# nintendops/EPN_PointCloud

Hardware: AMD Instinct MI355X
Metric: point-clouds/sec fwd+bwd, ModelNet40 N=1024 A=60 (higher is better)
Workload: dtype f32

## Files before the change

### epn_pointcloud_amd/csrc/c_api.hip

```cpp
#include <atomic>
#include <cstdlib>
#include <cstring>
#include <cxxabi.h>

#include "conv_internal.h"

using namespace epn;

static std::atomic<int> g_policy{0};
static bool force_generic() { return g_policy.load(std::memory_order_relaxed) == 1; }

namespace epn {
bool first_layer_on_valu() { return g_policy.load(std::memory_order_relaxed) == 2; }
#ifdef EPN_TUNING
int kernel_policy() { return g_policy.load(std::memory_order_relaxed); }
#else
int kernel_policy() { return 0; }
#endif
}

namespace {
thread_local const void *t_stub = nullptr;
thread_local bool t_stub_aux = true;
}
namespace epn {
void note_kernel(const void *host_stub, bool aux) {
    if (aux && t_stub) return;
    t_stub = host_stub;
    t_stub_aux = aux;
}
}

extern "C" const char *epn_last_kernel(void) {
    static thread_local char out[320];
    out[0] = 0;
    const void *stub = t_stub;
    t_stub = nullptr;
    t_stub_aux = true;
    if (!stub) return out;
    const char *mangled = hipKernelNameRefByPtr(stub, nullptr);
    if (!mangled) return out;
    int status = 0;
    char *dem = abi::__cxa_demangle(mangled, nullptr, nullptr, &status);
    const char *b = (status == 0 && dem) ? dem : mangled;
    if (!std::strncmp(b, "void ", 5)) b += 5;
    static const char anon[] = "(anonymous namespace)::";
    size_t o = 0;
    int depth = 0;
    for (size_t i = 0; b[i] && o + 1 < sizeof(out);) {
        if (!std::strncmp(b + i, anon, sizeof(anon) - 1)) { i += sizeof(anon) - 1; continue; }
        if (b[i] == '<') ++depth;
        else if (b[i] == '>') --depth;
        else if (b[i] == '(' && depth == 0) break;
        out[o++] = b[i++];
    }
    out[o] = 0;
    std::free(dem);
    return out;
}

extern "C" int epn_set_kernel_policy(int policy) {
#ifdef EPN_TUNING
    if (policy != 0 && policy != 1 && policy != 2 && (policy & ~0xff) != 0x100 && (policy & ~0xff) != 0x200 && (policy & ~0xff) != 0x400 && (policy & ~0xff) != 0x800 && (policy & ~0xff) != 0x900) return EPN_EINVAL;
#else
    if (policy != 0 && policy != 1 && policy != 2) return EPN_EINVAL;
#endif
    g_policy.store(policy, std::memory_order_relaxed);
    return 0;
}

static int check_desc(const epn_inter_desc *d) {
    if (!d) return EPN_ENULL;
    if (d->b < 0 || d->p1 < 1 || d->p2 < 0 || d->nn < 1 || d->na < 1 || d->ks < 1 || d->cin < 1 || d->cout < 1)
        return EPN_EINVAL;
    if (d->ks > EPN_KS_GENERIC_MAX) return EPN_EINVAL;
    if (!(d->sigma > 0.f) && !d->dense_w) return EPN_EINVAL;
    if (!d->ball_idx) return EPN_ENULL;
    if (!d->dense_w && (!d->xyz || !d->new_xyz || !d->anchors || !d->kernels)) return EPN_ENULL;
    return 0;
}

static bool use_mfma(const epn_inter_desc *d) { return inter_uses_mfma(d) && !force_generic() && !d->dense_w; }

extern "C" const char *epn_version(void) { return "epn_so3conv 0.5 (gfx950)"; }
extern "C" int epn_abi_version(void) { return EPN_ABI_VERSION; }

extern "C" const char *epn_strerror(int code) {
    switch (code) {
        case 0: return "success";
        case EPN_EINVAL: return "epn: invalid size or unsupported shape";
        case EPN_EWORKSPACE: return "epn: workspace missing or too small";
        case EPN_ENULL: return "epn: required pointer is NULL";
        default: return code > 0 ? hipGetErrorString((hipError_t)code) : "epn: unknown error";
    }
}

extern "C" int epn_inter_is_fused(const epn_inter_desc *d) {
    return d && (use_mfma(d) || (inter_c1_fwd_ok(d) && !force_generic())) ? 1 : 0;
}

extern "C" int epn_intra_is_fused(int na, int kn, int cin, int cout) {
    return intra_uses_mfma(na, kn, cin, cout) && !force_generic() ? 1 : 0;
}

extern "C" size_t epn_inter_workspace_bytes(const epn_inter_desc *d) {
    if (!d) return 0;
    InterWs w = inter_ws(d);
    if (force_generic() || d->dense_w) {
        epn_inter_desc g = *d;
        g.cin = d->cin; g.cout = d->cout;
        const size_t big = (size_t)d->b * d->p2 * d->na * d->cin * d->ks;
        return (w.big_off + rnd64(big)) * sizeof(float);
    }
    return w.total_floats * sizeof(float);
}

static int prep(const epn_inter_desc *d, void *workspace, size_t bytes, bool need_big, InterWs &ws, float *&base,
                hipStream_t st, bool need_rk = true) {
    int rc = check_desc(d);
    if (rc) return rc;
    ws = inter_ws(d);
    const size_t big = need_big ? rnd64((size_t)d->b * d->p2 * d->na * d->cin * d->ks)
                                : ws.total_floats - ws.big_off;
    if (!workspace || bytes < (ws.big_off + big) * sizeof(float)) return EPN_EWORKSPACE;
    base = static_cast<float *>(workspace);
    if (!d->dense_w && need_rk) {
        rc = launch_rk_table(d, base + ws.rk_off, st);
        if (rc) return rc;
    }
    return 0;
}

extern "C" int epn_inter_weights_f32(const epn_inter_desc *d, float *w, epn_stream_t stream) {
    int rc = check_desc(d);
    if (rc) return rc;
    if (!w || !d->xyz || !d->new_xyz || !d->anchors || !d->kernels) return EPN_ENULL;
    if (d->b == 0 || d->p2 == 0) return 0;
    return launch_inter_weights(d, w, epn_stream(stream));
}

extern "C" int epn_inter_so3conv_fwd_f32(const epn_inter_desc *d, const float *feats_cl, const float *W,
                                         float *out_cl, void *workspace, size_t workspace_bytes,
                                         epn_stream_t stream) {
    hipStream_t st = epn_stream(stream);
    InterWs ws;
    float *base = nullptr;
    const bool mf = d && use_mfma(d);
    int rc = prep(d, workspace, workspace_bytes, !mf, ws, base, st, !mf);
    if (rc) return rc;
    if (!feats_cl || !W || !out_cl) return EPN_ENULL;
    if (d->b == 0 || d->p2 == 0) return 0;
    if (mf) {
        rc = launch_inter_tables_mfma(d, base + ws.rk4_off, st);
        if (rc) return rc;
        return launch_inter_fwd_mfma(d, base + ws.rk4_off, feats_cl, W, out_cl, st);
    }
    if (inter_c1_fwd_ok(d) && !force_generic())
        return launch_inter_c1_fwd(d, base + ws.rk_off, feats_cl, W, out_cl, st, nullptr,
                                   reinterpret_cast<unsigned *>(base + ws.beta_off));
    float *G = base + ws.big_off;
    rc = launch_inter_group(d, base + ws.rk_off, feats_cl, G, st);
    if (rc) return rc;
    return launch_rowgemm_nt(G, W, (size_t)d->b * d->p2 * d->na, d->cin * d->ks, d->cout, out_cl, st);
}

extern "C" int epn_inter_c1_ok(const epn_inter_desc *d) {
    return d && !check_desc(d) && inter_c1_fwd_ok(d) && inter_c1_bwd_weight_ok(d) && !force_generic() ? 1 : 0;
}
extern "C" int epn_inter_so3conv_fwd_c1_f32(const epn_inter_desc *d, const float *feats_cl, const float *W, float *out_cl,
                                            float *grouped, void *workspace, size_t workspace_bytes, epn_stream_t stream) {
    if (!epn_inter_c1_ok(d)) return EPN_EINVAL;
    hipStream_t st = epn_stream(stream);
    InterWs ws;
    float *base = nullptr;
    int rc = prep(d, workspace, workspace_bytes, false, ws, base, st);
    if (rc) return rc;
    if (!feats_cl || !W || !out_cl) return EPN_ENULL;
    if (d->b == 0 || d->p2 == 0) return 0;
    return launch_inter_c1_fwd(d, base + ws.rk_off, feats_cl, W, out_cl, st, grouped,
                               reinterpret_cast<unsigned *>(base + ws.beta_off));
}
extern "C" int epn_inter_so3conv_bwd_weight_c1_f32(const epn_inter_desc *d, const float *grouped, const float *grad_out_cl,
                                                   float *grad_W, epn_stream_t stream) {
    if (!epn_inter_c1_ok(d)) return EPN_EINVAL;
    if (!grad_W) return EPN_ENULL;
    hipStream_t st = epn_stream(stream);
    EPN_HIP(hipMemsetAsync(grad_W, 0, sizeof(float) * (size_t)d->cout * d->ks, st));
    if (d->b == 0 || d->p2 == 0) return 0;
    if (!grouped || !grad_out_cl) return EPN_ENULL;
    return launch_inter_c1_bwd_weight(d, nullptr, nullptr, grad_out_cl, grad_W, st, grouped);
}

extern "C" int epn_inter_so3conv_bwd_data_f32(const epn_inter_desc *d, const float *grad_out_cl, const float *W,
                                              float *grad_feats_cl, void *workspace, size_t workspace_bytes,
                                              epn_stream_t stream) {
    hipStream_t st = epn_stream(stream);
    InterWs ws;
    float *base = nullptr;
    const bool mf = d && use_mfma(d);
    int rc = prep(d, workspace, workspace_bytes, !mf, ws, base, st, !mf);
    if (rc) return rc;
    if (!grad_feats_cl) return EPN_ENULL;
    EPN_HIP(hipMemsetAsync(grad_feats_cl, 0, sizeof(float) * (size_t)d->b * d->p1 * d->na * d->cin, st));
    if (d->b == 0 || d->p2 == 0) return 0;
    if (!grad_out_cl || !W) return EPN_ENULL;
    if (mf) {
        rc = launch_inter_tables_mfma(d, base + ws.rk4_off, st);
        if (rc) return rc;
        return launch_inter_bwd_data_mfma(d, base + ws.rk4_off, base + ws.big_off, grad_out_cl, W, grad_feats_cl, st);
    }
    float *dG = base + ws.big_off;
    rc = launch_rowgemm_nn(grad_out_cl, W, (size_t)d->b * d->p2 * d->na, d->cin * d->ks, d->cout, dG, st);
    if (rc) return rc;
    return launch_inter_scatter(d, base + ws.rk_off, dG, grad_feats_cl, st);
}

extern "C" int epn_inter_so3conv_bwd_weight_f32(const epn_inter_desc *d, const float *feats_cl,
                                                const float *grad_out_cl, float *grad_W, void *workspace,
                                                size_t workspace_bytes, epn_stream_t stream) {
    hipStream_t st = epn_stream(stream);
    InterWs ws;
    float *base = nullptr;
    const bool mf = d && use_mfma(d);
    int rc = prep(d, workspace, workspace_bytes, !mf, ws, base, st, !mf);
    if (rc) return rc;
    if (!grad_W) return EPN_ENULL;
    EPN_HIP(hipMemsetAsync(grad_W, 0, sizeof(float) * (size_t)d->cout * d->cin * d->ks, st));
    if (d->b == 0 || d->p2 == 0) return 0;
    if (!feats_cl || !grad_out_cl) return EPN_ENULL;
    if (mf) {
        rc = launch_inter_tables_mfma(d, base + ws.rk4_off, st);
        if (rc) return rc;
        return launch_inter_bwd_weight_mfma(d, base + ws.rk4_off, feats_cl, grad_out_cl, grad_W, st);
    }
    if (inter_c1_bwd_weight_ok(d) && !force_generic())
        return launch_inter_c1_bwd_weight(d, base + ws.rk_off, feats_cl, grad_out_cl, grad_W, st);
    float *G = base + ws.big_off;
    rc = launch_inter_group(d, base + ws.rk_off, feats_cl, G, st);
    if (rc) return rc;
    return launch_colreduce_dw(grad_out_cl, G, (size_t)d->b * d->p2 * d->na, d->cin * d->ks, d->cout, grad_W, st);
}

extern "C" size_t epn_inter_group_workspace_bytes(const epn_inter_desc *d) {
    if (!d) return 0;
    InterWs w = inter_ws(d);
    return w.big_off * sizeof(float);
}

static int prep_tables(const epn_inter_desc *d, void *workspace, size_t bytes, InterWs &ws, float *&base,
                       hipStream_t st, bool need_rk = true) {
    int rc = check_desc(d);
    if (rc) return rc;
    if (d->dense_w) return EPN_EINVAL;
    ws = inter_ws(d);
    if (!workspace || bytes < ws.big_off * sizeof(float)) return EPN_EWORKSPACE;
    base = static_cast<float *>(workspace);
    return need_rk ? launch_rk_table(d, base + ws.rk_off, st) : 0;
}

extern "C" int epn_inter_onchip_ok(const epn_inter_desc *d, int bf16) {
    return d && !check_desc(d) && inter_fx_ok(d, bf16) && !force_generic() ? 1 : 0;
}

extern "C" size_t epn_inter_onchip_workspace_bytes(const epn_inter_desc *d, int bf16) {
    if (!d) return 0;
    InterWs w = inter_ws(d);
    return w.big_off * sizeof(float) + inter_fx_planes_bytes(d, bf16);
}

static int inter_onchip_fwd(const epn_inter_desc *d, const void *feats_cl, const float *W, void *out_cl, void *workspace,
                            size_t workspace_bytes, int bf16, epn_stream_t stream) {
    hipStream_t st = epn_stream(stream);
    int rc = check_desc(d);
    if (rc) return rc;
    if (!inter_fx_ok(d, bf16)) return EPN_EINVAL;
    if (workspace_bytes < epn_inter_onchip_workspace_bytes(d, bf16)) return EPN_EWORKSPACE;
    InterWs ws;
    float *base = nullptr;
    rc = prep_tables(d, workspace, workspace_bytes, ws, base, st, false);
    if (rc) return rc;
    if (d->b == 0 || d->p2 == 0) return 0;
    if (!feats_cl || !W || !out_cl) return EPN_ENULL;
    rc = launch_inter_tables_mfma(d, base + ws.rk4_off, st);
    if (rc) return rc;
    return launch_inter_fx_fwd(d, base + ws.rk4_off, feats_cl, W, out_cl, base + ws.big_off, bf16, st);
}

extern "C" int epn_inter_so3conv_fwd_onchip_f32(const epn_inter_desc *d, const float *feats_cl, const float *W,
                                                float *out_cl, void *workspace, size_t workspace_bytes,
                                                epn_stream_t stream) {
    return inter_onchip_fwd(d, feats_cl, W, out_cl, workspace, workspace_bytes, 0, stream);
}
extern "C" int epn_inter_so3conv_fwd_bf16(const epn_inter_desc *d, const void *feats_cl, const float *W, void *out_cl,
                                          void *workspace, size_t workspace_bytes, epn_stream_t stream) {
    return inter_onchip_fwd(d, feats_cl, W, out_cl, workspace, workspace_bytes, 1, stream);
}

static int inter_group_any(const epn_inter_desc *d, const void *feats_cl, void *grouped, void *workspace,
                           size_t workspace_bytes, int bf16, epn_stream_t stream, int packed = 0) {
    hipStream_t st = epn_stream(stream);
    InterWs ws;
    float *base = nullptr;
    int rc = prep_tables(d, workspace, workspace_bytes, ws, base, st, !(d && inter_group_mfma_ok(d) && !force_generic()));
    if (rc) return rc;
    if (d->b == 0 || d->p2 == 0) return 0;
    if (!feats_cl || !grouped) return EPN_ENULL;
    if (inter_group_mfma_ok(d) && !force_generic()) {
        rc = launch_inter_tables_mfma(d, base + ws.rk4_off, st);
        if (rc) return rc;
        return launch_inter_group_mfma(d, base + ws.rk4_off, feats_cl, grouped, bf16, st, packed);
    }
    if (bf16 || packed) return EPN_EINVAL;
    return launch_inter_group(d, base + ws.rk_off, static_cast<const float *>(feats_cl), static_cast<float *>(grouped), st);
}

static int inter_ungroup_any(const epn_inter_desc *d, const void *grad_grouped, float *grad_feats_cl, void *workspace,
                             size_t workspace_bytes, int bf16, epn_stream_t stream, bool accumulate = false) {
    hipStream_t st = epn_stream(stream);
    InterWs ws;
    float *base = nullptr;
    int rc = prep_tables(d, workspace, workspace_bytes, ws, base, st, !(d && inter_group_mfma_ok(d) && !force_generic()));
    if (rc) return rc;
    if (!grad_feats_cl) return EPN_ENULL;
    if (!accumulate)
        EPN_HIP(hipMemsetAsync(grad_feats_cl, 0, sizeof(float) * (size_t)d->b * d->p1 * d->na * d->cin, st));
    if (d->b == 0 || d->p2 == 0) return 0;
    if (!grad_grouped) return EPN_ENULL;
    if (inter_group_mfma_ok(d) && !force_generic()) {
        rc = launch_inter_tables_mfma(d, base + ws.rk4_off, st);
        if (rc) return rc;
        return launch_inter_ungroup_mfma(d, base + ws.rk4_off, grad_grouped, grad_feats_cl,
                                         reinterpret_cast<int32_t *>(base + ws.order_off), bf16, st);
    }
    if (bf16) return EPN_EINVAL;
    return launch_inter_scatter(d, base + ws.rk_off, static_cast<const float *>(grad_grouped), grad_feats_cl, st);
}

extern "C" int epn_inter_group_f32(const epn_inter_desc *d, const float *feats_cl, float *grouped, void *workspace,
                                   size_t workspace_bytes, epn_stream_t stream) {
    return inter_group_any(d, feats_cl, grouped, workspace, workspace_bytes, 0, stream);
}
extern "C" int epn_inter_group_bf16(const epn_inter_desc *d, const void *feats_cl, void *grouped, void *workspace,
                                    size_t workspace_bytes, epn_stream_t stream) {
    return inter_group_any(d, feats_cl, grouped, workspace, workspace_bytes, 1, stream);
}
extern "C" int epn_inter_group_packed_ok(const epn_inter_desc *d) {
    return d && !check_desc(d) && inter_group_packed_ok(d) && !force_generic() ? 1 : 0;
}
extern "C" int epn_inter_packed_position(int cin, int ks, int32_t *position) {
    if (cin < 32 || cin % 32 || ks < 4 || ks > EPN_KS_MAX || ks % 4) return EPN_EINVAL;
    if (!position) return EPN_ENULL;
    for (int c = 0; c < cin; ++c)
        for (int k = 0; k < ks; ++k) position[c * ks + k] = inter_packed_position(c, k, cin, ks);
    return 0;
}
extern "C" int epn_inter_group_packed_f32(const epn_inter_desc *d, const float *feats_cl, float *grouped, void *workspace,
                                          size_t workspace_bytes, epn_stream_t stream) {
    if (!epn_inter_group_packed_ok(d)) return EPN_EINVAL;
    return inter_group_any(d, feats_cl, grouped, workspace, workspace_bytes, 0, stream, 1);
}
extern "C" int epn_inter_group_packed_bf16(const epn_inter_desc *d, const void *feats_cl, void *grouped, void *workspace,
                                           size_t workspace_bytes, epn_stream_t stream) {
    if (!epn_inter_group_packed_ok(d)) return EPN_EINVAL;
    return inter_group_any(d, feats_cl, grouped, workspace, workspace_bytes, 1, stream, 1);
}
static int pack_args_ok(int cout, int cin, int ks) {
    return cout >= 0 && cin >= 32 && cin % 32 == 0 && ks >= 4 && ks <= EPN_KS_MAX && ks % 4 == 0;
}
// ... 224 lines not shown
```

### epn_pointcloud_amd/csrc/epn_common.h

```cpp
#pragma once
#include <hip/hip_runtime.h>
#include <stdint.h>

#include "../../include/epn_so3conv.h"

#define EPN_WAVE 64

#define EPN_CHECK_LAUNCH()                         \
    do {                                           \
        hipError_t _e = hipGetLastError();         \
        if (_e != hipSuccess) return (int)_e;      \
    } while (0)

#define EPN_HIP(call)                              \
    do {                                           \
        hipError_t _e = (call);                    \
        if (_e != hipSuccess) return (int)_e;      \
    } while (0)

static inline hipStream_t epn_stream(epn_stream_t s) { return (hipStream_t)s; }

namespace epn {
void note_kernel(const void *host_stub, bool aux);
bool first_layer_on_valu();
}
#define EPN_LAUNCH(kern, ...)                                                       \
    do {                                                                            \
        ::epn::note_kernel(reinterpret_cast<const void *>(&kern), false);           \
        hipLaunchKernelGGL(kern, __VA_ARGS__);                                      \
    } while (0)
#define EPN_LAUNCH_AUX(kern, ...)                                                   \
    do {                                                                            \
        ::epn::note_kernel(reinterpret_cast<const void *>(&kern), true);            \
        hipLaunchKernelGGL(kern, __VA_ARGS__);                                      \
    } while (0)

static inline int epn_cdiv(long long a, long long b) { return (int)((a + b - 1) / b); }

__device__ __forceinline__ float epn_sq3(float a, float b, float c) {
    float t = __fmul_rn(a, a);
    t = __fmaf_rn(b, b, t);
    t = __fmaf_rn(c, c, t);
    return t;
}

__device__ __forceinline__ unsigned epn_xcd_tile(unsigned bid, unsigned nb) {
    const unsigned xcd = bid & 7u, local = bid >> 3;
    const unsigned q = nb >> 3, r = nb & 7u;
    return (xcd < r ? xcd * (q + 1) : r * (q + 1) + (xcd - r) * q) + local;
}

typedef float f32x4 __attribute__((ext_vector_type(4)));
typedef float f32x16 __attribute__((ext_vector_type(16)));
```

### epn_pointcloud_amd/csrc/inter_ungroup_cloud.hip

```cpp
#include "inter_device.h"
#include "gemm.h"

namespace epn {
namespace {

__device__ unsigned g_uc_range = 0u;

constexpr int UC_DUMMY = 4;
constexpr int UC_LDS_MAX = 160 * 1024;

constexpr int UC_PTS = 8;
__global__ __launch_bounds__(256) void uc_slots_kernel(const int32_t *__restrict__ idx, const float *__restrict__ xyz,
                                                       const float *__restrict__ new_xyz, long long npts, int p1, int p2, int nn, int ew,
                                                       float sigma_inv, unsigned rowb, uint32_t *__restrict__ off,
                                                       float *__restrict__ hood, unsigned *__restrict__ mulmax) {
    const int lane = threadIdx.x & 63;
    const long long pt0 = ((long long)blockIdx.x * 4 + (threadIdx.x >> 6)) * UC_PTS;
    if (pt0 >= npts) return;
    const bool in = lane < nn;
    int q[UC_PTS];
#pragma unroll
    for (int i = 0; i < UC_PTS; ++i) {
        const long long pt = pt0 + i < npts ? pt0 + i : npts - 1;
        q[i] = in ? idx[pt * nn + lane] : -1;
    }
    bool valid[UC_PTS];
    unsigned mul[UC_PTS];
    float g[UC_PTS][3], cc[UC_PTS][3];
#pragma unroll
    for (int i = 0; i < UC_PTS; ++i) {
        const long long pt = pt0 + i < npts ? pt0 + i : npts - 1;
        const long long bb = pt / p2;
        const int pp = (int)(pt - bb * p2);
        const int first = __shfl(q[i], 0, 64);
        const unsigned long long rep = __ballot(in && lane > 0 && q[i] == first);
        int cnt = rep ? (int)__builtin_ctzll(rep) : nn;
        const int qprev = __shfl(q[i], lane >= cnt ? lane - cnt : lane, 64);
        const bool bad = in && lane >= cnt && q[i] != qprev;
        if (__ballot(bad) != 0ull) cnt = nn;
        valid[i] = q[i] >= 0 && q[i] < p1;
        mul[i] = (valid[i] && lane < cnt) ? (unsigned)((nn - 1 - lane) / cnt + 1) : 0u;
        const float *s = xyz + bb * 3 * p1, *c = new_xyz + bb * 3 * p2;
        const int qq = valid[i] ? q[i] : 0;
        g[i][0] = s[qq]; g[i][1] = s[p1 + qq]; g[i][2] = s[2 * p1 + qq];
        cc[i][0] = c[pp]; cc[i][1] = c[p2 + pp]; cc[i][2] = c[2 * p2 + pp];
    }
    unsigned m = 0;
#pragma unroll
    for (int i = 0; i < UC_PTS; ++i) {
        const long long pt = pt0 + i < npts ? pt0 + i : npts - 1;
        if (lane < ew) {
            off[pt * ew + lane] = (valid[i] ? (unsigned)q[i] : (unsigned)(p1 + ((lane >> 2) & 3))) * rowb;
            const float gx = g[i][0] - cc[i][0], gy = g[i][1] - cc[i][1], gz = g[i][2] - cc[i][2];
            const float alpha = 1.0f - (gx * gx + gy * gy + gz * gz) * sigma_inv;
            const float mf = (float)mul[i];
            float *h = hood + pt * 5 * ew + lane;
            h[0] = gx * mf; h[ew] = gy * mf; h[2 * ew] = gz * mf; h[3 * ew] = mf; h[4 * ew] = alpha * mf;
        }
        m = mul[i] > m ? mul[i] : m;
    }
#pragma unroll
    for (int o = 32; o >= 1; o >>= 1) {
        const unsigned v = (unsigned)__shfl_xor((int)m, o, 64);
        m = v > m ? v : m;
    }
    if (lane == 0 && m > 1u && m > __atomic_load_n(mulmax, __ATOMIC_RELAXED)) atomicMax(mulmax, m);
}

template <typename TG>
__global__ __launch_bounds__(256) void uc_absmax_kernel(const TG *__restrict__ src, long long n, unsigned *__restrict__ out) {
    unsigned m = 0;
    for (long long i = (long long)blockIdx.x * 256 + threadIdx.x; i < n; i += (long long)gridDim.x * 256) {
        unsigned a;
        if constexpr (sizeof(TG) == 2) a = ((unsigned)__builtin_bit_cast(unsigned short, src[i]) & 0x7fffu) << 16;
        else a = __builtin_bit_cast(unsigned, src[i]) & 0x7fffffffu;
        m = (a > m && a < 0x7f800000u) ? a : m;
    }
#pragma unroll
    for (int o = 32; o >= 1; o >>= 1) {
        const unsigned v = (unsigned)__shfl_xor((int)m, o, 64);
        m = v > m ? v : m;
    }
    if ((threadIdx.x & 63) == 0 && m > __atomic_load_n(out, __ATOMIC_RELAXED)) atomicMax(out, m);
}

struct UcArgs {
    InterArgs A;
    const uint32_t *tab;
    const float *hood;
    const unsigned *mulmax;
    const float *dg_amax;
    const void *add;
    int cr;
    int out_bf16;
};

typedef unsigned u32x4_t __attribute__((ext_vector_type(4)));
typedef unsigned u32x2_t __attribute__((ext_vector_type(2)));

__device__ __forceinline__ float uc_scale(float amax, unsigned mulmax, int ks) {
    unsigned e = (__builtin_bit_cast(unsigned, amax) >> 23) & 255u;
    e = e < 1u ? 1u : e;
    const unsigned f = (mulmax < 1u ? 1u : mulmax) * (unsigned)ks;
    const int bits = f > 1u ? 32 - __builtin_clz(f - 1u) : 0;
    int se = 127 + 50 - bits - ((int)e - 126);
    se = se < 1 ? 1 : (se > 240 ? 240 : se);
    return __builtin_bit_cast(float, (unsigned)se << 23);
}

template <int NT, int KT, typename TG, int NWV, int NL>
__global__ __launch_bounds__(64 * NWV) void inter_ungroup_cloud_kernel(UcArgs P) {
    extern __shared__ __attribute__((aligned(16))) char uc_smem[];
    const InterArgs &A = P.A;
    constexpr int EW = 16 * NT;
    constexpr int NTH = 64 * NWV;
    constexpr int CR = 16 * NL;
    constexpr unsigned ROWB = CR * 8u;
    typedef typename std::conditional<sizeof(TG) == 2, bf16x4_t, f32x4>::type frag_t;

    const int tid = threadIdx.x;
    const int lane = tid & 63;
    const int wave = __builtin_amdgcn_readfirstlane(tid >> 6);
    const int x = lane & 15, j = lane >> 4;
    const int blk = epn_xcd_tile(blockIdx.x, gridDim.x);
    const int bb = blk / A.na, a = blk - bb * A.na;
    const int c0 = blockIdx.y * CR;
    const int rows = A.p1 + UC_DUMMY;
    int *poison = reinterpret_cast<int *>(uc_smem + (size_t)rows * ROWB);

    {
        const u32x4_t z = {0u, 0u, 0u, 0u};
        u32x4_t *acc4 = reinterpret_cast<u32x4_t *>(uc_smem);
        for (int i = tid; i < rows * (CR / 2); i += NTH) acc4[i] = z;
        if (tid == 0) *poison = 0;
    }
    const float S = uc_scale(*P.dg_amax, *P.mulmax, A.ks);
    const float invS = __builtin_bit_cast(float, (254u - (__builtin_bit_cast(unsigned, S) >> 23)) << 23);
    float rk[KT];
#pragma unroll
    for (int kt = 0; kt < KT; ++kt) rk[kt] = A.rk4[((size_t)a * EPN_KS_MAX + 16 * kt + x) * 4 + j];
    const int gss = A.cin * A.ks;
    const uint32_t *tabc = P.tab + (size_t)bb * A.p2 * EW + 4 * j;
    const float *hoodc = P.hood + (size_t)bb * A.p2 * 5 * EW + j * EW + x;
    const TG *dGc = reinterpret_cast<const TG *>(A.gout) + ((size_t)bb * A.p2 * A.na + a) * gss + (size_t)(c0 + x) * A.ks;
    int koff[KT];
#pragma unroll
    for (int kt = 0; kt < KT; ++kt) koff[kt] = 16 * kt + 4 * (16 * kt + 4 * j < A.ks ? j : 0);
    auto load_dg = [&](int p, int cw, frag_t (&d)[KT]) {
        const TG *src = dGc + (size_t)p * A.na * gss + (size_t)(16 * cw) * A.ks;
#pragma unroll
        for (int kt = 0; kt < KT; ++kt) {
            if constexpr (sizeof(TG) == 2) d[kt] = *reinterpret_cast<const bf16x4_t *>(src + koff[kt]);
            else d[kt] = ld4f(src + koff[kt]);
        }
    };
    auto load_tab = [&](int p, float (&hb)[NT], float (&ha)[NT], u32x4_t (&e4)[NT]) {
        const uint32_t *t0 = tabc + (size_t)p * EW;
        const float *h0 = hoodc + (size_t)p * 5 * EW;
#pragma unroll
        for (int t = 0; t < NT; ++t) {
            hb[t] = h0[16 * t];
            ha[t] = h0[16 * t + (4 - j) * EW];
            e4[t] = *reinterpret_cast<const u32x4_t *>(t0 + 16 * t);
        }
    };
    __syncthreads();

    typedef __attribute__((address_space(3))) char lds_char;
    typedef __attribute__((address_space(3))) unsigned long long lds_u64;
    const unsigned x8b = (unsigned)(uintptr_t)(lds_char *)uc_smem + 8u * (unsigned)x;
    int chkp = 0;
    unsigned chkn = 0u;
    if (wave < A.p2) {
        float hbn[NT], han[NT];
        u32x4_t e4n[NT];
        constexpr int D = sizeof(TG) == 2 ? NL : (NL < 4 ? NL : 4);
        frag_t ring[D][KT];
        load_tab(wave, hbn, han, e4n);
#pragma unroll
        for (int i = 0; i < D; ++i) load_dg(wave, i, ring[i]);
        for (int p = wave; p < A.p2; p += NWV) {
            float gB[NT], alphaN[NT];
            unsigned rowoff[NT][4];
#pragma unroll
            for (int t = 0; t < NT; ++t) {
                gB[t] = hbn[t] * S;
                alphaN[t] = han[t] * S;
#pragma unroll
                for (int r = 0; r < 4; ++r) rowoff[t][r] = e4n[t][r] + x8b;
            }
            const int pn = p + NWV < A.p2 ? p + NWV : p;
            load_tab(pn, hbn, han, e4n);
            frag_t wgt[NT][KT];
#pragma unroll
            for (int t = 0; t < NT; ++t) {
#pragma unroll
                for (int kt = 0; kt < KT; ++kt) {
                    f32x4 sk = {alphaN[t], alphaN[t], alphaN[t], alphaN[t]};
                    sk = mfma4(rk[kt], gB[t], sk);
                    if constexpr (sizeof(TG) == 2) {
                        wgt[t][kt] = relu_pack4(sk);
                    } else {
#pragma unroll
                        for (int r = 0; r < 4; ++r) sk[r] = relu_f(sk[r]);
                        wgt[t][kt] = sk;
                    }
                }
            }
#pragma unroll
            for (int cw = 0; cw < NL; ++cw) {
                frag_t dgc[KT];
#pragma unroll
                for (int kt = 0; kt < KT; ++kt) dgc[kt] = ring[cw % D][kt];
                if (cw + D < NL) load_dg(p, cw + D, ring[cw % D]);
                else load_dg(pn, cw + D - NL, ring[cw % D]);
                f32x4 tt[NT];
#pragma unroll
                for (int t = 0; t < NT; ++t) {
                    tt[t] = f32x4{0.f, 0.f, 0.f, 0.f};
                    if constexpr (sizeof(TG) == 2) {
                        if constexpr (KT == 2) tt[t] = mfma_bf16_k32(wgt[t][0], wgt[t][1], dgc[0], dgc[1], tt[t]);
                        else tt[t] = mfma_bf16_k16(wgt[t][0], dgc[0], tt[t]);
                    } else {
#pragma unroll
                        for (int kt = 0; kt < KT; ++kt)
#pragma unroll
                            for (int r = 0; r < 4; ++r) tt[t] = mfma4(wgt[t][kt][r], dgc[kt][r], tt[t]);
                    }
                }
#pragma unroll
                for (int t = 0; t < NT; ++t)
#pragma unroll
                    for (int r = 0; r < 4; ++r) {
                        const float v = tt[t][r];
                        const unsigned vb = __builtin_bit_cast(unsigned, v);
                        chkp = (int)vb > chkp ? (int)vb : chkp;
                        chkn = vb > chkn ? vb : chkn;
                        const double dv = (double)v + 6755399441055744.0;
                        u32x2_t w = __builtin_bit_cast(u32x2_t, dv);
                        w[1] -= 0x43380000u;
                        lds_u64 *dst = (lds_u64 *)(uintptr_t)(rowoff[t][r] + (unsigned)cw * 128u);
                        __hip_atomic_fetch_add((unsigned long long *)dst, __builtin_bit_cast(unsigned long long, w), __ATOMIC_RELAXED,
                                               __HIP_MEMORY_SCOPE_WORKGROUP);
                    }
            }
        }
    }
    if (__builtin_amdgcn_ballot_w64(chkp >= 0x58800000 || chkn >= 0xd8800000u) != 0ull && lane == 0) {
        atomicAdd(&g_uc_range, 1u);
        *poison = 1;
    }
    __syncthreads();
    const float bad = *poison ? __builtin_nanf("") : 0.0f;

    const long long *acc = reinterpret_cast<const long long *>(uc_smem);
    const size_t obase = ((size_t)bb * A.p1 * A.na + a) * A.cin + c0;
    const size_t ostride = (size_t)A.na * A.cin;
    constexpr int CR2 = CR / 2;
    for (int i = tid; i < A.p1 * CR2; i += NTH) {
        const int q = i / CR2, c = 2 * (i - q * CR2);
        const long long v0 = acc[q * CR + c], v1 = acc[q * CR + c + 1];
        float f0 = (float)v0 * invS + bad, f1 = (float)v1 * invS + bad;
        const size_t o = obase + (size_t)q * ostride + c;
        if (P.out_bf16) {
            typedef __bf16 bf16x2_t __attribute__((ext_vector_type(2)));
            if (P.add) {
                const bf16x2_t ad = *reinterpret_cast<const bf16x2_t *>(static_cast<const __bf16 *>(P.add) + o);
                f0 += (float)ad[0]; f1 += (float)ad[1];
            }
            *reinterpret_cast<bf16x2_t *>(reinterpret_cast<__bf16 *>(A.out) + o) = bf16x2_t{(__bf16)f0, (__bf16)f1};
        } else {
            if (P.add) {
                const float2 ad = *reinterpret_cast<const float2 *>(static_cast<const float *>(P.add) + o);
                f0 += ad.x; f1 += ad.y;
            }
            *reinterpret_cast<float2 *>(A.out + o) = make_float2(f0, f1);
        }
    }
}

size_t uc_lds_bytes(const epn_inter_desc *d, int cr) { return (size_t)(d->p1 + UC_DUMMY) * cr * 8 + 16; }

int uc_channels_per_wg(const epn_inter_desc *d, int bf16) {
    int best = 0;
    const int cap = d->nn > 32 ? (bf16 ? 64 : 16) : ((!bf16 && d->nn > 16) ? 64 : 128);
    for (int cr = 16; cr <= cap && cr <= d->cin; cr *= 2)
        if (d->cin % cr == 0 && uc_lds_bytes(d, cr) <= (size_t)UC_LDS_MAX) best = cr;
    return best;
}

template <typename K>
int uc_set_lds(K kern, size_t bytes) {
    return (int)hipFuncSetAttribute(reinterpret_cast<const void *>(kern), hipFuncAttributeMaxDynamicSharedMemorySize, (int)bytes);
}

}

long long ungroup_cloud_range_take(bool reset) {
    unsigned v = 0;
    hipError_t e = hipMemcpyFromSymbol(&v, HIP_SYMBOL(g_uc_range), sizeof(v), 0, hipMemcpyDeviceToHost);
    if (e != hipSuccess) return -(long long)e;
    if (reset && v) {
        const unsigned zero = 0;
        e = hipMemcpyToSymbol(HIP_SYMBOL(g_uc_range), &zero, sizeof(zero), 0, hipMemcpyHostToDevice);
        if (e != hipSuccess) return -(long long)e;
    }
    return (long long)v;
}

bool inter_ungroup_cloud_ok(const epn_inter_desc *d) {
    if (!inter_group_mfma_ok(d)) return false;
    return d->na >= 1 && d->nn <= 64 && d->ks <= 32 && d->p1 + UC_DUMMY <= 65536 && d->p2 <= 4096 && d->cin % 16 == 0 &&
           uc_channels_per_wg(d, 0) > 0 && (long long)d->b * d->p2 * d->na * d->cin * d->ks < (1LL << 40);
}

static size_t uc_off_bytes(const epn_inter_desc *d) {
    const int nt = d->nn <= 16 ? 1 : (d->nn <= 32 ? 2 : 4);
    return ((size_t)d->b * d->p2 * 16 * nt * 4 + 255) & ~(size_t)255;
}
size_t inter_ungroup_cloud_extra_bytes(const epn_inter_desc *d) {
    const int nt = d->nn <= 16 ? 1 : (d->nn <= 32 ? 2 : 4);
    return uc_off_bytes(d) + (((size_t)d->b * d->p2 * nt * 80 * 4 + 255) & ~(size_t)255) + 256;
}

int launch_inter_ungroup_cloud(const epn_inter_desc *d, const float *rk4, const void *dG, const float *dg_amax, void *dF,
                               const void *add, int bf16, int out_bf16, void *extra, hipStream_t st) {
    const int nt = d->nn <= 16 ? 1 : (d->nn <= 32 ? 2 : 4), ew = 16 * nt;
    uint32_t *tab = static_cast<uint32_t *>(extra);
    unsigned *mulmax = reinterpret_cast<unsigned *>(static_cast<char *>(extra) + inter_ungroup_cloud_extra_bytes(d) - 256);
    EPN_HIP(hipMemsetAsync(mulmax, 0, 8, st));
    if (!dg_amax) {
        unsigned *slot = mulmax + 1;
        const long long n = (long long)d->b * d->p2 * d->na * d->cin * d->ks;
        const unsigned nb = (unsigned)((n + 256 * 16 - 1) / (256 * 16) < 8192 ? (n + 256 * 16 - 1) / (256 * 16) : 8192);
        if (bf16) EPN_LAUNCH_AUX(uc_absmax_kernel<__bf16>, dim3(nb ? nb : 1), dim3(256), 0, st, static_cast<const __bf16 *>(dG), n, slot);
        else EPN_LAUNCH_AUX(uc_absmax_kernel<float>, dim3(nb ? nb : 1), dim3(256), 0, st, static_cast<const float *>(dG), n, slot);
        EPN_CHECK_LAUNCH();
        dg_amax = reinterpret_cast<const float *>(slot);
    }
    const long long npts = (long long)d->b * d->p2;
    float *hood = reinterpret_cast<float *>(static_cast<char *>(extra) + uc_off_bytes(d));
    EPN_LAUNCH_AUX(uc_slots_kernel, dim3((unsigned)((npts + 4 * UC_PTS - 1) / (4 * UC_PTS))), dim3(256), 0, st, d->ball_idx, d->xyz, d->new_xyz, npts, d->p1, d->p2,
                   d->nn, ew, 1.0f / d->sigma, (unsigned)uc_channels_per_wg(d, bf16) * 8u, tab, hood, mulmax);
    EPN_CHECK_LAUNCH();
    UcArgs P;
    InterArgs &A = P.A;
    A.xyz = d->xyz; A.new_xyz = d->new_xyz; A.idx = d->ball_idx; A.rk4 = rk4;
    A.feats = nullptr; A.W = nullptr; A.gout = static_cast<const float *>(dG); A.out = static_cast<float *>(dF);
    A.sigma_inv = 1.0f / d->sigma;
    A.b = d->b; A.p1 = d->p1; A.p2 = d->p2; A.nn = d->nn; A.na = d->na; A.ks = d->ks; A.cin = d->cin; A.cout = d->cout;
    A.wk = 0; A.packed = 0; A.ncol = (long long)d->b * d->p2 * d->na; A.col_tiles_per_wg = 1;
    P.tab = tab; P.hood = hood; P.mulmax = mulmax; P.dg_amax = dg_amax; P.add = add; P.out_bf16 = out_bf16;
    P.cr = uc_channels_per_wg(d, bf16);
    const size_t lds = uc_lds_bytes(d, P.cr);
    const dim3 grid((unsigned)(d->b * d->na), (unsigned)(d->cin / P.cr));
    const int kt = (d->ks + 15) / 16, nl = P.cr / 16;
    int rc = 0;
#define EPN_UC(NT_, KT_, TG_, NL_)                                                                                   \
    do {                                                                                                             \
        rc = uc_set_lds(inter_ungroup_cloud_kernel<NT_, KT_, TG_, 16, NL_>, lds);                                    \
        if (rc) return rc;                                                                                           \
        EPN_LAUNCH((inter_ungroup_cloud_kernel<NT_, KT_, TG_, 16, NL_>), grid, dim3(64 * 16), lds, st, P);           \
    } while (0)
#define EPN_UC_L(NT_, KT_, TG_)                                                                                      \
    do {                                                                                                             \
        if (nl == 1) EPN_UC(NT_, KT_, TG_, 1); else if (nl == 2) EPN_UC(NT_, KT_, TG_, 2);                           \
        else if (nl == 4) EPN_UC(NT_, KT_, TG_, 4); else EPN_UC(NT_, KT_, TG_, 8);                                   \
    } while (0)
#define EPN_UC_T(NT_, KT_)                                                                                           \
    do {                                                                                                             \
        if (bf16) EPN_UC_L(NT_, KT_, __bf16); else EPN_UC_L(NT_, KT_, float);                                        \
    } while (0)
    if (kt == 1) {
        if (nt == 1) EPN_UC_T(1, 1); else if (nt == 2) EPN_UC_T(2, 1); else EPN_UC_T(4, 1);
    } else {
        if (nt == 1) EPN_UC_T(1, 2); else if (nt == 2) EPN_UC_T(2, 2); else EPN_UC_T(4, 2);
    }
#undef EPN_UC_T
#undef EPN_UC_L
#undef EPN_UC
    EPN_CHECK_LAUNCH();
    return 0;
}

}
```

Measured before the change: 537.3.

## Add two-workgroup-per-CU plan for ungroup-cloud kernel with 8-wave blocks

Adds a planning helper that, for medium neighbourhood sizes, picks an 8-wave workgroup with half the LDS budget. This lets two workgroups share a CU instead of one 16-wave block holding all of its LDS. In that form the per-wave dG prefetch ring is restructured so each wave unrolls over several points. The ring depth and slot indexing now span point boundaries. Tuning-only flags to skip the main loop or the output stage are also added. The risks are smaller channel tiles per workgroup, more workgroups, and extra register pressure from the deeper ring under the new launch-bounds hint.

```diff
diff --git a/epn_pointcloud_amd/csrc/c_api.hip b/epn_pointcloud_amd/csrc/c_api.hip
--- a/epn_pointcloud_amd/csrc/c_api.hip
+++ b/epn_pointcloud_amd/csrc/c_api.hip
@@ -12,6 +12,7 @@
 
 namespace epn {
 bool first_layer_on_valu() { return g_policy.load(std::memory_order_relaxed) == 2; }
+bool ungroup_cloud_one_wg() { return g_policy.load(std::memory_order_relaxed) == 3; }
 #ifdef EPN_TUNING
 int kernel_policy() { return g_policy.load(std::memory_order_relaxed); }
 #else
@@ -61,9 +62,9 @@
 
 extern "C" int epn_set_kernel_policy(int policy) {
 #ifdef EPN_TUNING
-    if (policy != 0 && policy != 1 && policy != 2 && (policy & ~0xff) != 0x100 && (policy & ~0xff) != 0x200 && (policy & ~0xff) != 0x400 && (policy & ~0xff) != 0x800 && (policy & ~0xff) != 0x900) return EPN_EINVAL;
+    if (policy != 0 && policy != 1 && policy != 2 && policy != 3 && (policy & ~0xff) != 0x100 && (policy & ~0xff) != 0x200 && (policy & ~0xff) != 0x400 && (policy & ~0xff) != 0x800 && (policy & ~0xff) != 0x900 && (policy & ~0xff) != 0xa00) return EPN_EINVAL;
 #else
-    if (policy != 0 && policy != 1 && policy != 2) return EPN_EINVAL;
+    if (policy != 0 && policy != 1 && policy != 2 && policy != 3) return EPN_EINVAL;
 #endif
     g_policy.store(policy, std::memory_order_relaxed);
     return 0;
diff --git a/epn_pointcloud_amd/csrc/epn_common.h b/epn_pointcloud_amd/csrc/epn_common.h
--- a/epn_pointcloud_amd/csrc/epn_common.h
+++ b/epn_pointcloud_amd/csrc/epn_common.h
@@ -23,6 +23,7 @@
 namespace epn {
 void note_kernel(const void *host_stub, bool aux);
 bool first_layer_on_valu();
+bool ungroup_cloud_one_wg();
 }
 #define EPN_LAUNCH(kern, ...)                                                       \
     do {                                                                            \
diff --git a/epn_pointcloud_amd/csrc/inter_ungroup_cloud.hip b/epn_pointcloud_amd/csrc/inter_ungroup_cloud.hip
--- a/epn_pointcloud_amd/csrc/inter_ungroup_cloud.hip
+++ b/epn_pointcloud_amd/csrc/inter_ungroup_cloud.hip
@@ -1,13 +1,11 @@
 #include "inter_device.h"
 #include "gemm.h"
+#include "ungroup_cloud_plan.h"
 
 namespace epn {
 namespace {
 
 __device__ unsigned g_uc_range = 0u;
-
-constexpr int UC_DUMMY = 4;
-constexpr int UC_LDS_MAX = 160 * 1024;
 
 constexpr int UC_PTS = 8;
 __global__ __launch_bounds__(256) void uc_slots_kernel(const int32_t *__restrict__ idx, const float *__restrict__ xyz,
@@ -109,7 +107,7 @@
 }
 
 template <int NT, int KT, typename TG, int NWV, int NL>
-__global__ __launch_bounds__(64 * NWV) void inter_ungroup_cloud_kernel(UcArgs P) {
+__global__ __launch_bounds__(64 * NWV, 4) void inter_ungroup_cloud_kernel(UcArgs P) {
     extern __shared__ __attribute__((aligned(16))) char uc_smem[];
     const InterArgs &A = P.A;
     constexpr int EW = 16 * NT;
@@ -126,6 +124,11 @@
     const int bb = blk / A.na, a = blk - bb * A.na;
     const int c0 = blockIdx.y * CR;
     const int rows = A.p1 + UC_DUMMY;
+#ifdef EPN_TUNING
+    const bool skip_main = (A.wk & 1) != 0, skip_out = (A.wk & 2) != 0;
+#else
+    constexpr bool skip_main = false, skip_out = false;
+#endif
     int *poison = reinterpret_cast<int *>(uc_smem + (size_t)rows * ROWB);
 
     {
@@ -171,15 +174,24 @@
     const unsigned x8b = (unsigned)(uintptr_t)(lds_char *)uc_smem + 8u * (unsigned)x;
     int chkp = 0;
     unsigned chkn = 0u;
-    if (wave < A.p2) {
+    if (wave < A.p2 && !skip_main) {
         float hbn[NT], han[NT];
         u32x4_t e4n[NT];
-        constexpr int D = sizeof(TG) == 2 ? NL : (NL < 4 ? NL : 4);
+        constexpr int D = NWV == 16 ? (sizeof(TG) == 2 ? NL : (NL < 4 ? NL : 4)) : (NL < 4 ? 4 : (sizeof(TG) == 2 ? NL : 4));
+        constexpr int U = D > NL ? D / NL : 1;
+        static_assert(D % NL == 0 || NL % D == 0, "ring slots are static");
         frag_t ring[D][KT];
         load_tab(wave, hbn, han, e4n);
 #pragma unroll
-        for (int i = 0; i < D; ++i) load_dg(wave, i, ring[i]);
-        for (int p = wave; p < A.p2; p += NWV) {
+        for (int i = 0; i < D; ++i) {
+            const int pt = wave + (i / NL) * NWV;
+            load_dg(pt < A.p2 ? pt : wave, i % NL, ring[i]);
+        }
+        for (int p0 = wave; p0 < A.p2; p0 += NWV * U) {
+#pragma unroll
+          for (int u = 0; u < U; ++u) {
+            const int p = p0 + u * NWV;
+            if (p >= A.p2) break;
             float gB[NT], alphaN[NT];
             unsigned rowoff[NT][4];
 #pragma unroll
@@ -211,9 +223,11 @@
             for (int cw = 0; cw < NL; ++cw) {
                 frag_t dgc[KT];
 #pragma unroll
-                for (int kt = 0; kt < KT; ++kt) dgc[kt] = ring[cw % D][kt];
-                if (cw + D < NL) load_dg(p, cw + D, ring[cw % D]);
-                else load_dg(pn, cw + D - NL, ring[cw % D]);
+                for (int kt = 0; kt < KT; ++kt) dgc[kt] = ring[(u * NL + cw) % D][kt];
+                {
+                    const int pt = p + ((cw + D) / NL) * NWV;
+                    load_dg(pt < A.p2 ? pt : p, (cw + D) % NL, ring[(u * NL + cw) % D]);
+                }
                 f32x4 tt[NT];
 #pragma unroll
                 for (int t = 0; t < NT; ++t) {
@@ -244,6 +258,7 @@
                                                __HIP_MEMORY_SCOPE_WORKGROUP);
                     }
             }
+          }
         }
     }
     if (__builtin_amdgcn_ballot_w64(chkp >= 0x58800000 || chkn >= 0xd8800000u) != 0ull && lane == 0) {
@@ -257,7 +272,7 @@
     const size_t obase = ((size_t)bb * A.p1 * A.na + a) * A.cin + c0;
     const size_t ostride = (size_t)A.na * A.cin;
     constexpr int CR2 = CR / 2;
-    for (int i = tid; i < A.p1 * CR2; i += NTH) {
+    for (int i = tid; i < (skip_out ? 0 : A.p1 * CR2); i += NTH) {
         const int q = i / CR2, c = 2 * (i - q * CR2);
         const long long v0 = acc[q * CR + c], v1 = acc[q * CR + c + 1];
         float f0 = (float)v0 * invS + bad, f1 = (float)v1 * invS + bad;
@@ -279,14 +294,10 @@
     }
 }
 
-size_t uc_lds_bytes(const epn_inter_desc *d, int cr) { return (size_t)(d->p1 + UC_DUMMY) * cr * 8 + 16; }
-
-int uc_channels_per_wg(const epn_inter_desc *d, int bf16) {
-    int best = 0;
-    const int cap = d->nn > 32 ? (bf16 ? 64 : 16) : ((!bf16 && d->nn > 16) ? 64 : 128);
-    for (int cr = 16; cr <= cap && cr <= d->cin; cr *= 2)
-        if (d->cin % cr == 0 && uc_lds_bytes(d, cr) <= (size_t)UC_LDS_MAX) best = cr;
-    return best;
+UcPlan uc_plan_of(const epn_inter_desc *d, int bf16) {
+    int form = ungroup_cloud_one_wg() ? 16 : 0;
+    if ((kernel_policy() & 0xf00) == 0xa00) form = (kernel_policy() & 4) ? 16 : ((kernel_policy() & 8) ? 8 : form);
+    return uc_plan(d->p1, d->p2, d->nn, d->ks, d->cin, bf16, form);
 }
 
 template <typename K>
@@ -310,8 +321,8 @@
 
 bool inter_ungroup_cloud_ok(const epn_inter_desc *d) {
     if (!inter_group_mfma_ok(d)) return false;
-    return d->na >= 1 && d->nn <= 64 && d->ks <= 32 && d->p1 + UC_DUMMY <= 65536 && d->p2 <= 4096 && d->cin % 16 == 0 &&
-           uc_channels_per_wg(d, 0) > 0 && (long long)d->b * d->p2 * d->na * d->cin * d->ks < (1LL << 40);
+    return d->na >= 1 && uc_plan(d->p1, d->p2, d->nn, d->ks, d->cin, 0, 0).cr > 0 &&
+           (long long)d->b * d->p2 * d->na * d->cin * d->ks < (1LL << 40);
 }
 
 static size_t uc_off_bytes(const epn_inter_desc *d) {
@@ -339,9 +350,11 @@
         dg_amax = reinterpret_cast<const float *>(slot);
     }
     const long long npts = (long long)d->b * d->p2;
+    const UcPlan plan = uc_plan_of(d, bf16);
+    if (plan.cr == 0) return EPN_EINVAL;
     float *hood = reinterpret_cast<float *>(static_cast<char *>(extra) + uc_off_bytes(d));
     EPN_LAUNCH_AUX(uc_slots_kernel, dim3((unsigned)((npts + 4 * UC_PTS - 1) / (4 * UC_PTS))), dim3(256), 0, st, d->ball_idx, d->xyz, d->new_xyz, npts, d->p1, d->p2,
-                   d->nn, ew, 1.0f / d->sigma, (unsigned)uc_channels_per_wg(d, bf16) * 8u, tab, hood, mulmax);
+                   d->nn, ew, 1.0f / d->sigma, (unsigned)plan.cr * 8u, tab, hood, mulmax);
     EPN_CHECK_LAUNCH();
     UcArgs P;
     InterArgs &A = P.A;
@@ -351,21 +364,27 @@
     A.b = d->b; A.p1 = d->p1; A.p2 = d->p2; A.nn = d->nn; A.na = d->na; A.ks = d->ks; A.cin = d->cin; A.cout = d->cout;
     A.wk = 0; A.packed = 0; A.ncol = (long long)d->b * d->p2 * d->na; A.col_tiles_per_wg = 1;
     P.tab = tab; P.hood = hood; P.mulmax = mulmax; P.dg_amax = dg_amax; P.add = add; P.out_bf16 = out_bf16;
-    P.cr = uc_channels_per_wg(d, bf16);
-    const size_t lds = uc_lds_bytes(d, P.cr);
+    P.cr = plan.cr;
+    const size_t lds = plan.lds;
+#ifdef EPN_TUNING
+    if ((kernel_policy() & 0xf00) == 0xa00) A.wk = kernel_policy() & 3;
+#endif
     const dim3 grid((unsigned)(d->b * d->na), (unsigned)(d->cin / P.cr));
     const int kt = (d->ks + 15) / 16, nl = P.cr / 16;
     int rc = 0;
-#define EPN_UC(NT_, KT_, TG_, NL_)                                                                                   \
+#define EPN_UC(NT_, KT_, TG_, NWV_, NL_)                                                                             \
     do {                                                                                                             \
-        rc = uc_set_lds(inter_ungroup_cloud_kernel<NT_, KT_, TG_, 16, NL_>, lds);                                    \
+        rc = uc_set_lds(inter_ungroup_cloud_kernel<NT_, KT_, TG_, NWV_, NL_>, lds);                                  \
         if (rc) return rc;                                                                                           \
-        EPN_LAUNCH((inter_ungroup_cloud_kernel<NT_, KT_, TG_, 16, NL_>), grid, dim3(64 * 16), lds, st, P);           \
+        EPN_LAUNCH((inter_ungroup_cloud_kernel<NT_, KT_, TG_, NWV_, NL_>), grid, dim3(64 * NWV_), lds, st, P);       \
     } while (0)
 #define EPN_UC_L(NT_, KT_, TG_)                                                                                      \
     do {                                                                                                             \
-        if (nl == 1) EPN_UC(NT_, KT_, TG_, 1); else if (nl == 2) EPN_UC(NT_, KT_, TG_, 2);                           \
-        else if (nl == 4) EPN_UC(NT_, KT_, TG_, 4); else EPN_UC(NT_, KT_, TG_, 8);                                   \
+        if (plan.nwv == 8) {                                             \
+            if (nl == 1) EPN_UC(NT_, KT_, TG_, 8, 1); else if (nl == 2) EPN_UC(NT_, KT_, TG_, 8, 2);                 \
+            else EPN_UC(NT_, KT_, TG_, 8, 4);                                                                        \
+        } else if (nl == 1) EPN_UC(NT_, KT_, TG_, 16, 1); else if (nl == 2) EPN_UC(NT_, KT_, TG_, 16, 2);            \
+        else if (nl == 4) EPN_UC(NT_, KT_, TG_, 16, 4); else EPN_UC(NT_, KT_, TG_, 16, 8);                           \
     } while (0)
 #define EPN_UC_T(NT_, KT_)                                                                                           \
     do {                                                                                                             \
diff --git a/epn_pointcloud_amd/csrc/ungroup_cloud_plan.h b/epn_pointcloud_amd/csrc/ungroup_cloud_plan.h
--- /dev/null
+++ b/epn_pointcloud_amd/csrc/ungroup_cloud_plan.h
@@ -0,0 +1,39 @@
+#pragma once
+#include <cstddef>
+
+namespace epn {
+
+constexpr int UC_DUMMY = 4;
+constexpr int UC_LDS_MAX = 160 * 1024;
+constexpr int UC_NN_MAX = 64, UC_KS_MAX = 32, UC_P2_MAX = 4096;
+
+struct UcPlan {
+    int nwv;
+    int cr;
+    int wgs;
+    size_t lds;
+};
+
+inline size_t uc_lds_bytes(int p1, int cr) { return (size_t)(p1 + UC_DUMMY) * cr * 8 + 16; }
+
+inline int uc_channels(int p1, int nn, int cin, int bf16, size_t lds_max, int cr_max) {
+    int best = 0;
+    int cap = nn > 32 ? (bf16 ? 64 : 16) : ((!bf16 && nn > 16) ? 64 : 128);
+    cap = cap < cr_max ? cap : cr_max;
+    for (int cr = 16; cr <= cap && cr <= cin; cr *= 2)
+        if (cin % cr == 0 && uc_lds_bytes(p1, cr) <= lds_max) best = cr;
+    return best;
+}
+
+inline UcPlan uc_plan(int p1, int p2, int nn, int ks, int cin, int bf16, int form) {
+    UcPlan none = {0, 0, 0, 0};
+    if (p1 < 1 || p2 < 0 || p2 > UC_P2_MAX || nn < 1 || nn > UC_NN_MAX || ks < 4 || ks > UC_KS_MAX || ks % 4 != 0 || cin < 16 || cin % 16 != 0) return none;
+    const int cr16 = uc_channels(p1, nn, cin, bf16, UC_LDS_MAX, 128);
+    if (cr16 == 0) return none;
+    const int cr8 = uc_channels(p1, nn, cin, bf16, UC_LDS_MAX / 2, 64);
+    const bool two = form == 8 || (form == 0 && nn > 16 && (bf16 ? cr8 >= 64 : nn <= 32));
+    if (two && cr8 > 0) return UcPlan{8, cr8, 2, uc_lds_bytes(p1, cr8)};
+    return UcPlan{16, cr16, 1, uc_lds_bytes(p1, cr16)};
+}
+
+}
```

Result: no change. 538.0 (median of 4 runs) (+0.1%).
